# electrum/presto

Measured on AMD Instinct MI355X. Metric: rows/s through operator pipeline, TPC-H Q1+Q6 SF100, 1/2/4/8 GPUs vs CPU ref, higher is better.
Workload: dtype f64

## Files before the change

### presto_amd/csrc/op_fused.cpp

```cpp
#include <algorithm>
#include <cstring>
#include <sstream>

#include "op_fused.hpp"

namespace pa {
namespace fused_op {

FusedAggregationOperator::FusedAggregationOperator(const pa_fused_aggregation_desc* d)
    : FusedAggregationOperator(make_spec(d), d->aggregation.stream ? d->aggregation.stream : d->filter_project.stream)
{
}

FusedAggregationOperator::FusedAggregationOperator(Spec spec, void* stream) : spec_(std::move(spec)), stream_(stream)
{
    require_device();
    nullable_seen_.assign(spec_.n_in, false);
    out_partial_ = spec_.step == PA_STEP_PARTIAL;
    {
        std::ostringstream f;
        for (int c = 0; c < spec_.n_in; c++) f << spec_.in_types[c] << ',' << spec_.in_params[c] << ';';
        f << '|' << (spec_.has_filter ? spec_.filter.fingerprint() : std::string("-")) << '|';
        for (const auto& p : spec_.proj) f << p.fingerprint() << '#';
        f << '|';
        for (int g : spec_.group_proj) f << g << ',';
        f << '|' << spec_.hash_channel << '|' << spec_.step << '|';
        for (const auto& a : spec_.aggs) f << a.fn << ',' << a.input_channel << ',' << a.mask_channel << ',' << a.input_type << ';';
        if (spec_.join) {
            f << "|join:" << spec_.join->key_proj << ':';
            for (int32_t t : spec_.join->build_types) f << t << ',';
            f << ':';
            for (int j : spec_.join->brow_group_proj) f << j << ',';
        }
        f << "|lds_pipe:" << lds_pipe_level();
        plan_fingerprint_ = f.str();
    }
    grouped_ = !spec_.group_proj.empty();
    mode_ = grouped_ ? (spec_.expected_groups > (1 << 20) ? V_GT : V_LDS) : V_GLOBAL;
    if (spec_.any_ranked() && grouped_) mode_ = V_GT;
    cus_ = device_cu_count();
    ctl_ = static_cast<int32_t*>(ctl_buf_.ensure(64));
    PA_HIP(hipMemsetAsync(ctl_, 0, 64, stream_.get()));
    h_ctl_ = static_cast<int32_t*>(h_ctl_buf_.ensure(256));
    memset(h_ctl_, 0, 256);
}

FusedAggregationOperator::~FusedAggregationOperator()
{
    (void)hipStreamSynchronize(stream_.get());
    if (lds_.merge_stream) pool_stream_release(lds_.merge_stream);
    release_everything();
    for (hipEvent_t e : release_events_) (void)hipEventDestroy(e);
    for (int b = 0; b < 2; b++) {
        if (arena_[b].table_event) (void)hipEventDestroy(arena_[b].table_event);
        if (arena_[b].vtable_event) (void)hipEventDestroy(arena_[b].vtable_event);
        if (lds_.ev_main[b]) (void)hipEventDestroy(lds_.ev_main[b]);
        if (lds_.ev_merge[b]) (void)hipEventDestroy(lds_.ev_merge[b]);
    }
    for (RangeTable& t : range_table_) {
        if (t.event) (void)hipEventDestroy(t.event);
    }
}

bool FusedAggregationOperator::set_output_topn(int64_t n, const int32_t* channels, const int32_t* orders, int32_t count)
{
    if (n <= 0 || count <= 0 || !grouped_ || out_partial_ || spec_.step == PA_STEP_PARTIAL) return false;
    topn_hint_.n = n;
    topn_hint_.channels.assign(channels, channels + count);
    topn_hint_.orders.assign(orders, orders + count);
    return true;
}

bool FusedAggregationOperator::retry_parked()
{
    if (!parked_) return true;
    if (!pool_has_room(parked_need_)) return false;
    parked_ = false;
    pa_page page = parked_page_;
    page.columns = parked_cols_.data();
    take_page(&page);
    return !parked_;
}

void FusedAggregationOperator::take_page(const pa_page* page)
{
    const uint64_t launched = timer.begun();
    try {
        if (next_) {
            next_->add_input(page);
            return;
        }
        cur_rel_set_ = (page->flags & PA_PAGE_RETAINED) != 0 && page->release != nullptr;
        cur_rel_ = Release{page->release, page->release_ctx};
        if (gather_small_page(page)) return;
        flush_pending();
        if (next_) {
            cur_rel_set_ = false;
            next_->add_input(page);
            return;
        }
        process_page(page, page_stays(page) && page->mem == PA_MEM_DEVICE);
        if (cur_rel_set_) {
            std::vector<Release> rel{cur_rel_};
            cur_rel_set_ = false;
            release_checkpoint(std::move(rel), true);
        }
    }
    catch (const PoolExhausted& e) {
        if (!page_stays(page) || timer.begun() != launched || is_combiner_) throw;
        parked_page_ = *page;
        if (!cur_rel_set_) parked_page_.flags &= ~PA_PAGE_RETAINED;
        cur_rel_set_ = false;
        parked_cols_.assign(page->columns, page->columns + page->channel_count);
        parked_need_ = e.bytes;
        parked_ = true;
    }
}

void FusedAggregationOperator::add_input(const pa_page* page)
{
    PA_REQUIRE(!finishing_, PA_ERR_ILLEGAL_STATE, "Operator is already finishing");
    PA_REQUIRE(page != nullptr, PA_ERR_INVALID_ARGUMENT, "page is null");
    PA_REQUIRE(page->channel_count == spec_.n_in, PA_ERR_INVALID_ARGUMENT, "page channel count does not match the operator's input types");
    poll_releases();
    if (page->position_count == 0) {
        if ((page->flags & PA_PAGE_RETAINED) != 0 && page->release) page->release(page->release_ctx);
        return;
    }
    PA_REQUIRE(!parked_, PA_ERR_ILLEGAL_STATE, "Operator has unfinished work");
    take_page(page);
}

void FusedAggregationOperator::process_page(const pa_page* page, bool retained)
{
    if (next_) {
        next_->process_page(page, retained);
        return;
    }
    retained_ = retained;
    try {
        add_page(page);
    }
    catch (const LayoutChange&) {
        start_next_generation();
        next_->process_page(page, retained);
    }
    retained_ = false;
}

void FusedAggregationOperator::start_next_generation()
{
    PA_REQUIRE(!is_combiner_ && generation_ <= spec_.n_in, PA_ERR_DEVICE, "internal: state layout changed more often than channels exist");
    confirm_all();
    next_ = std::make_unique<FusedAggregationOperator>(spec_, stream_.get());
    next_->nullable_seen_ = nullable_seen_;
    next_->generation_ = generation_ + 1;
}

void FusedAggregationOperator::finish()
{
    if (finishing_) return;
    PA_REQUIRE(retry_parked(), PA_ERR_INSUFFICIENT_RESOURCES, "finish while a page is still waiting for HBM: the pool's budget does not cover the aggregation");
    flush_pending();
    finishing_ = true;
    poll_releases();
}

bool FusedAggregationOperator::get_output(pa_page* out)
{
    poll_releases();
    if (!finishing_ || output_done_) return false;
    output_done_ = true;
    confirm_all();
    if (next_) return combine_generations(out);
    build_output();
    if (grouped_ && out_rows_ > 0) decode_interned_keys();
    if (!grouped_ || out_rows_ > 0) {
        publish_output(out_cols_, out_rows_, spec_.output_mem, stream_.get(), out, out_storage_);
        poll_releases();
        return true;
    }
    poll_releases();
    return false;
}

bool FusedAggregationOperator::emit_states(pa_page* out)
{
    flush_pending();
    confirm_all();
    out_partial_ = true;
    spec_.output_mem = PA_MEM_DEVICE;
    build_output();
    if (grouped_ && out_rows_ > 0) decode_interned_keys();
    if (grouped_ && out_rows_ == 0) return false;
    publish_output(out_cols_, out_rows_, PA_MEM_DEVICE, stream_.get(), out, out_storage_);
    return true;
}

bool FusedAggregationOperator::combine_generations(pa_page* out)
{
    Spec cs = combiner_spec();
    combiner_ = std::make_unique<FusedAggregationOperator>(std::move(cs), stream_.get());
    combiner_->out_partial_ = spec_.step == PA_STEP_PARTIAL;
    combiner_->nullable_seen_.assign(combiner_->spec_.n_in, true);
    combiner_->is_combiner_ = true;
    for (FusedAggregationOperator* g = this; g != nullptr; g = g->next_.get()) {
        pa_page states{};
        if (g->emit_states(&states)) combiner_->add_input(&states);
    }
    combiner_->finish();
    return combiner_->get_output(out);
}

Spec FusedAggregationOperator::combiner_spec() const
{
    Spec c;
    c.step = PA_STEP_FINAL;
    c.output_mem = spec_.output_mem;
    c.expected_groups = spec_.expected_groups;
    auto add_channel = [&](int32_t type, int32_t param) {
        c.in_types.push_back(type);
        c.in_params.push_back(param);
        OwnedExpr e;
        pa_expr_node node{};
        node.kind = PA_EXPR_INPUT_REF;
        node.type = type;
        node.channel = c.n_in;
        e.nodes.push_back(node);
        e.strings.emplace_back();
        e.root = 0;
        c.proj.push_back(std::move(e));
        return c.n_in++;
    };
    for (size_t gi = 0; gi < spec_.group_proj.size(); gi++) {
        const OwnedExpr& pe = spec_.proj[spec_.group_proj[gi]];
        int ch = pe.is_input_ref() ? pe.node(pe.root).channel : -1;
        if (ch >= spec_.n_in) ch = -1;
        const bool interned = ch >= 0 && spec_.interned[ch];
        c.group_proj.push_back(add_channel(interned ? (int32_t)PA_VARCHAR : pe.root_type(), ch >= 0 ? spec_.in_params[ch] : 0));
    }
    c.hash_channel = spec_.hash_channel >= 0 && !spec_.group_proj.empty() ? add_channel(PA_BIGINT, 0) : -1;
    for (const pa_aggregate& ag : spec_.aggs) {
        pa_aggregate f = ag;
        f.mask_channel = -1;
        f.input_channel = add_channel(PA_BIGINT, 0);
        if (ag.fn != PA_AGG_COUNT && ag.fn != PA_AGG_COUNT_STAR) {
            const int value_proj = spec_.step == PA_STEP_FINAL ? ag.input_channel + 1 : ag.input_channel;
            int32_t t = spec_.proj[value_proj].root_type();
            if (ag.fn == PA_AGG_AVG || (ag.fn == PA_AGG_SUM && t == PA_DOUBLE)) t = PA_DOUBLE;
// ... 180 lines not shown
```

### presto_amd/csrc/op_fused.hpp

```cpp
#pragma once

#include <atomic>
#include <deque>
#include <map>
#include <memory>
#include <mutex>
#include <string>
#include <vector>

#include "exchange_kernels.hpp"
#include "fused_plan.hpp"
#include "intern_kernels.hpp"
#include "jit.hpp"
#include "join_source.hpp"
#include "operator.hpp"
#include "scan_kernels.hpp"
#include "static_kernels.hpp"

namespace pa {

using namespace fused;

namespace fused_op {

// ... 29 lines not shown
        if (!retry_parked()) return true;
        if (next_) return next_->is_blocked();
        poll_inflight();
        return lds_.inflight.size() >= kMaxInflight;
    }
    void add_input(const pa_page* page) override;
    void finish() override;
    bool is_finished() override { return finishing_ && output_done_; }
    bool get_output(pa_page* out) override;
    bool set_output_topn(int64_t n, const int32_t* channels, const int32_t* orders, int32_t count) override;
    int64_t memory_bytes() override
    {
        return (int64_t)(stager_.bytes() + slab_.capacity() + gt_.tag.capacity() + gt_.keys.capacity() + gt_.words.capacity() + state_.capacity());
    }
    int64_t group_bytes();
    const Spec& spec() const { return spec_; }
    void* stream_handle() { return stream_.get(); }

private:
    struct TopNHint {
        int64_t n = 0;
        std::vector<int32_t> channels, orders;
    };
    struct Release {
        void (*fn)(void*) = nullptr;
        void* ctx = nullptr;
    };
    struct ReleaseBatch {
        hipEvent_t event = nullptr;
        uint64_t seq = 0;
        std::vector<Release> rel;
    };
    struct Compiled {
        KernelInfo info;
        JitKernel kernel, tail_kernel;
        DevBuf kinds;
        mutable std::atomic<int> lds_verdict{0};
        mutable std::atomic<int> staged_verdict{0};
    };
    struct RowList {
        const int32_t* rows;
        int64_t count;
        int64_t first_row;
        int64_t chunk_rows;
    };
    struct Inflight {
        int b = 0;
        DevPage dp;
        bool vec = false;
        int64_t offset = 0;
        std::string sig;
        std::vector<ChannelLayout> layout;
        uint64_t seq = 0;
    };
    struct Run {
        int64_t rows = 0;
        bool flat = true;
        std::vector<pa_column> cols;
    };
    struct RangeTable {
        PinnedBuf host;
        DevBuf dev;
        hipEvent_t event = nullptr;
        bool used = false;
    };
    struct Arena {
        int64_t rows = 0;
        std::vector<bool> nullable;
        std::vector<DevBuf> values, nulls, offsets;
        std::vector<int64_t> bytes;
        std::vector<CopySeg> segs;
        std::vector<Release> rel;
        PinnedBuf h_table;
        DevBuf d_table;
        hipEvent_t table_event = nullptr;
        bool table_used = false;
        bool dev_var = false, var_fresh = true;
        int cursor_half = 0;
        DevBuf cursors;
        std::vector<VarSeg> vsegs;
        PinnedBuf h_vtable;
        DevBuf d_vtable;
        hipEvent_t vtable_event = nullptr;
        bool vtable_used = false;
    };
    struct RankedChannel {
        std::vector<std::string> strings;
        std::vector<uint32_t> order;
        DevBuf ranks, image;
    };

    bool lookup_source_ready() const { return !spec_.join || spec_.join->ls->built.load(); }
    static bool page_stays(const pa_page* page) { return (page->flags & (PA_PAGE_STABLE | PA_PAGE_RETAINED)) != 0; }
    bool retry_parked();
    void take_page(const pa_page* page);
    void process_page(const pa_page* page, bool retained);
    void start_next_generation();
    bool emit_states(pa_page* out);
    bool combine_generations(pa_page* out);
    Spec combiner_spec() const;
    static void raise_if(int32_t code);

    Release take_cur_release()
    {
        cur_rel_set_ = false;
        return cur_rel_;
// ... 33 lines not shown
    static std::mutex& shared_mutex();
    static std::map<std::string, std::shared_ptr<const Compiled>>& shared_cache();
    const Compiled& kernel_for(const std::string& sig, const std::vector<ChannelLayout>& layout, int variant);
    void adopt_layout(const Compiled& c);
    static constexpr int64_t kStagedMinRows = (int64_t)1 << 22;
    static constexpr double kStagedGain = 0.85;
    static int staged_mode();
    const Compiled* staged_kernel(const std::string& sig, const std::vector<ChannelLayout>& layout, int64_t rows);
    static double staged_bytes(const std::vector<int>& w, const std::vector<double>& alive);
    void staged_decide(const Compiled& ck, const uint64_t* slab, int grid, int64_t vec_rows, hipStream_t s);
    bool run_page(const Compiled& ck, const DevPage& dp, bool vec, const RowList* list = nullptr, int64_t start_row = 0);
    void fill_join_args(FusedArgs& a) const;
    void advance_columns(FusedArgs& a, const DevPage& dp, int64_t offset) const;
    bool run_page_build_rows(const Compiled& ck, const DevPage& dp, FusedArgs a, int64_t start_row);
    bool launch_global(const Compiled& ck, const DevPage& dp, FusedArgs& a, int64_t offset, int64_t total, int64_t range_entries);
    bool launch_lds(const Compiled& ck, const DevPage& dp, FusedArgs& a, bool vec, int64_t offset, int64_t total, int64_t range_entries);
    bool launch_table(const Compiled& ck, const DevPage& dp, FusedArgs& a, const RowList* list, int64_t offset, int64_t total);
    int grid_for(const KernelInfo& ki, int64_t work, const RowList* list) const;
    uint32_t replicas_for(const KernelInfo& ki, int grid, const RowList* list) const;
    FusedArgs replay_args(const FusedArgs& a, uint32_t spilled, int cur, uint64_t flush_room);
    static constexpr size_t kMaxInflight = 2;
    int32_t* h_ctl_lds(int b) const { return h_ctl_ + 16 + 8 * b; }
    void poll_inflight();
    void confirm_all();
    void confirm_all_but_last();
    bool confirm_oldest(bool redo = true);

    static constexpr int64_t kProbeRows = (int64_t)1 << 18;
    static constexpr uint32_t kLdshReplicas = 4;
    static uint32_t desired_replicas(uint64_t g);
    void ensure_table(uint64_t min_groups, uint32_t reps = 0);
    static uint64_t estimate_groups(uint64_t d, uint64_t n);
    void drop_table();
    void read_group_counts(hipStream_t s);
    void drain_merges();
    bool partitioned_wanted(const std::string& sig, const std::vector<ChannelLayout>& layout, int* partitions);
    void run_page_partitioned(const std::string& sig, const std::vector<ChannelLayout>& layout, const DevPage& dp, bool vec, int partitions,
                              int64_t start_row);
    const uint64_t* table_tags() const
    {
        return build_rows_table_ && brow_occ_word_ >= 0 ? gt_.words.as<uint64_t>() + (size_t)brow_occ_word_ * gt_.cap : gt_.tag.as<uint64_t>();
    }
    const uint64_t* table_words() const { return gt_.words.as<uint64_t>(); }
    GtStrides table_strides() const { return GtStrides{1u, gt_.cap, 1u, 0u, build_rows_table_ && brow_occ_word_ >= 0 ? brow_occ_empty_ : 0ULL}; }

    void intern_keys(DevPage& dp, hipStream_t s);
    void intern_dictionary_key(const pa_page* page, int c, DevPage& dp, hipStream_t s);
    void decode_interned_keys();
    int interned_channel(int gi) const;
    void rank_values(DevPage& dp, hipStream_t s);
    void rerank_words(int c, const uint32_t* ranks, hipStream_t s);
    int ranked_channel(int proj) const;

    void build_output();
    bool emit_on_device(const KernelInfo& ki, int64_t groups, bool keys_from_build_columns = false);


    Spec spec_;
    Stream stream_;
    std::string plan_fingerprint_;
    bool grouped_ = false, finishing_ = false, output_done_ = false;
    int cus_ = 256;
    int mode_ = V_GLOBAL;
    DevBuf ctl_buf_;
    PinnedBuf h_ctl_buf_;
    int32_t* ctl_ = nullptr;
    int32_t* h_ctl_ = nullptr;

    TopNHint topn_hint_;
    bool out_partial_ = false;
    std::vector<bool> nullable_seen_;
    int generation_ = 0;
    bool is_combiner_ = false;
    std::unique_ptr<FusedAggregationOperator> next_;
    std::unique_ptr<FusedAggregationOperator> combiner_;
    bool parked_ = false;
    pa_page parked_page_{};
    std::vector<pa_column> parked_cols_;
    size_t parked_need_ = 0;

    PageStager stager_;
    PinnedPageCopy pinned_copy_;
    std::vector<int64_t> var_bytes_hint_;
    Release cur_rel_;
    bool cur_rel_set_ = false;
    std::vector<Release> run_rel_, ranges_rel_, carry_rel_;
    std::deque<ReleaseBatch> release_batches_;
    std::vector<hipEvent_t> release_events_;
    Run run_;
    std::shared_ptr<std::vector<DevPage>> ranges_;
    int64_t range_rows_ = 0;
    RangeTable range_table_[3];
    int range_table_next_ = 0;
    Arena arena_[2];
    int arena_cur_ = 0;

    std::map<std::string, std::shared_ptr<const Compiled>> compiled_;
    bool layout_fixed_ = false;
    int nw_ = 0, w_ = 0;
    std::string layout_id_;
    const int32_t* kinds_dev_ = nullptr;
    const KernelInfo* last_info_ = nullptr;
    bool staged_refused_ = false;
    bool join_checked_ = false;
    const std::string* cur_sig_ = nullptr;
    const std::vector<ChannelLayout>* cur_layout_ = nullptr;
    bool retained_ = false;
    int64_t resume_from_ = -1;

    DevBuf slab_, state_;

    struct LdsTier {
        DevBuf slab[2], entry_slot[2];
        hipStream_t merge_stream = nullptr;
        hipEvent_t ev_main[2] = {nullptr, nullptr}, ev_merge[2] = {nullptr, nullptr};
        bool merge_pending[2] = {false, false};
        int page = 0;
        bool probed = false;
        const Compiled* compiled = nullptr;
        std::deque<Inflight> inflight;
        uint64_t launch_seq = 0;
    } lds_;

    struct HbmTable {
        DevBuf tag, keys, words, rep_count, spill[2];
        PinnedBuf h_rep;
        uint32_t cap = 0, rep = 1;
        uint64_t groups_upper = 0, groups_sum = 0;
        uint64_t probed_groups = 0;
        bool probed = false;
    } gt_;
    bool build_rows_table_ = false;
    const Compiled* brow_keys_ = nullptr;
    int brow_occ_word_ = -1;
    uint64_t brow_occ_empty_ = 0;

    struct Partitioned {
        int parts = 0, lc = 0;
        bool want = false;
        bool fresh = false;
        uint64_t fell = 0;
        DevBuf tag, keys, words, count, part_first;
        DevBuf part_ids, part_pos, part_counts, part_temp;
        std::vector<DevBuf> reorder_bufs;
        int list_grid_hint = 0;
    } ldsp_;

    std::vector<std::unique_ptr<StringInterner>> interners_;
    PageStager dict_stager_;
    std::vector<DevBuf> dict_key_bufs_;
    std::vector<std::unique_ptr<RankedChannel>> ranked_;

    PinnedBuf h_table_, h_parts_;
    DevBuf dense_keys_, dense_words_, null_flags_;
    std::vector<OutColumn> out_cols_;
    std::vector<pa_column> out_storage_;
    int32_t out_rows_ = 0;
    static constexpr int64_t kHostDecodeGroups = 4096;
    static constexpr uint32_t kHostDecodeIds = 4096;
    std::vector<std::vector<std::string>> host_dict_;
};

}
}
```

### presto_amd/csrc/op_fused_launch.cpp

```cpp
#include <algorithm>
#include <cmath>
#include <cstring>

#include "op_fused.hpp"

namespace pa {
namespace fused_op {

void FusedAggregationOperator::add_page(const pa_page* page)
{
    HostTraceScope trace("  fused.add_page");
    hipStream_t s = stream_.get();
    std::vector<int> dict_keys;
    std::vector<bool> needed = spec_.used_channel;
    for (int c = 0; c < spec_.n_in; c++) {
        if (!spec_.interned[c]) continue;
        const pa_column& col = page->columns[c];
        const bool encoded = (col.encoding == PA_DICTIONARY && col.ids != nullptr) || col.encoding == PA_RLE;
        if (!encoded || col.dictionary == nullptr || col.dictionary->encoding != PA_VARWIDTH) continue;
        const int64_t dn = col.encoding == PA_RLE ? 1 : col.dictionary_size;
        if (dn <= 0 || dn > page->position_count) continue;
        needed[c] = false;
        dict_keys.push_back(c);
    }
// ... 212 lines not shown
    return true;
}

bool FusedAggregationOperator::launch_lds(const Compiled& ck, const DevPage& dp, FusedArgs& a, bool vec, int64_t offset, int64_t total,
                                          int64_t range_entries)
{
    hipStream_t s = stream_.get();
    const KernelInfo& ki = ck.info;
    const int64_t lds_head = dp.ranges ? total : vec ? (total & ~(int64_t)255) : 0;
    while (offset < total) {
        int64_t n = total - offset;
        bool use_tail = false;
        if (offset < lds_head) {
            n = lds_head - offset;
            if (!lds_.probed && ck.lds_verdict.load(std::memory_order_relaxed) == 1) lds_.probed = true;
            lds_.compiled = &ck;
            if (!lds_.probed && n > ((int64_t)1 << 22) && !dp.ranges) n = (int64_t)1 << 20;
        }
        else use_tail = true;
        advance_columns(a, dp, offset);
        a.n = n;
        int64_t work = use_tail ? n : (n + 3) / 4;
        if (dp.ranges) work = range_entries * ki.block;
        const int per_cu = std::max(1, std::min(16, (int)(160 * 1024 / ((size_t)ki.nw * ki.c * 64 * 8 + 512))));
        const int grid = std::max((int)std::min<int64_t>((work + 63) / 64, (int64_t)cus_ * per_cu), 1);
        const int b = lds_.page & 1;
        if (!lds_.merge_stream) {
            lds_.merge_stream = pool_stream_acquire();
            for (int i = 0; i < 2; i++) {
                PA_HIP(hipEventCreateWithFlags(&lds_.ev_main[i], hipEventDisableTiming));
                PA_HIP(hipEventCreateWithFlags(&lds_.ev_merge[i], hipEventDisableTiming));
            }
        }
        while (lds_.inflight.size() >= kMaxInflight) confirm_oldest();
        if (mode_ != V_LDS) {
            resume_from_ = offset;
            return false;
        }
        if (lds_.merge_pending[b]) PA_HIP(hipStreamWaitEvent(s, lds_.ev_merge[b], 0));
        a.slab = static_cast<uint64_t*>(lds_.slab[b].ensure((size_t)grid * ki.c * (1 + ki.w + ki.nw) * 8));
        a.overflow_rows = reinterpret_cast<uint64_t*>(ctl_ + 2 + 2 * b);
        ensure_table(gt_.groups_upper + 2 * (uint64_t)grid * ki.c);
        a.gt_tag = gt_.tag.as<uint64_t>();
        a.gt_keys = gt_.keys.as<uint64_t>();
        a.gt_words = gt_.words.as<uint64_t>();
        a.gt_mask = gt_.cap ? gt_.cap - 1 : 0;
        a.gt_max_fill = (int32_t)(gt_.cap - gt_.cap / 4);
        a.gt_rep_count = gt_.rep_count.as<int32_t>();
        void* params[] = {&a};
        if (!use_tail) timer.set_name(ck.kernel.name);
        timer.begin(s);
        PA_HIP(hipModuleLaunchKernel(use_tail ? ck.tail_kernel.fn : ck.kernel.fn, grid, 1, 1, ki.block, 1, 1, 0, s, params, nullptr));
        timer.end(s, !use_tail);
        PA_HIP(hipMemcpyAsync(h_ctl_lds(b), ctl_, 32, hipMemcpyDeviceToHost, s));
        PA_HIP(hipEventRecord(lds_.ev_main[b], s));
        PA_HIP(hipStreamWaitEvent(lds_.merge_stream, lds_.ev_main[b], 0));
        launch_merge_lds_slab(a.slab, grid, ki.c, ki.w, ki.nw, ck.kinds.as<int32_t>(), a.gt_tag, a.gt_keys, a.gt_words, a.gt_mask,
                              a.gt_max_fill, a.gt_count, ctl_, a.overflow_rows,
                              static_cast<int32_t*>(lds_.entry_slot[b].ensure((size_t)grid * ki.c * 4)), lds_.merge_stream);
        PA_HIP(hipEventRecord(lds_.ev_merge[b], lds_.merge_stream));
        lds_.merge_pending[b] = true;
        lds_.page++;
        Inflight f;
        f.b = b;
        f.dp = dp;
        f.dp.n = (int32_t)(offset + n);
        f.vec = vec;
        f.offset = offset;
        f.sig = *cur_sig_;
        f.layout = *cur_layout_;
        f.seq = ++lds_.launch_seq;
        lds_.inflight.push_back(std::move(f));
        if (!lds_.probed) {
            confirm_all_but_last();
            if (!confirm_oldest(false)) {
                resume_from_ = offset;
                return false;
            }
        }
        else if (!retained_) confirm_all();
        else poll_inflight();
        if (mode_ != V_LDS) {
            resume_from_ = offset + n;
            return false;
        }
        offset += n;
        if (resume_from_ >= 0) return false;
    }
    return true;
}

int FusedAggregationOperator::grid_for(const KernelInfo& ki, int64_t work, const RowList* list) const
{
    int grid;
    if (ki.variant == V_LDSP) {
        grid = ldsp_.parts;
    }
    else if (ki.variant == V_LDSH) {
        grid = (int)std::min<int64_t>((work + ki.block - 1) / ki.block, (int64_t)cus_ * (ki.block == 1024 ? 1 : 2));
        if (list && ldsp_.list_grid_hint > grid) grid = (int)std::min<int64_t>((work + ki.block - 1) / ki.block, (int64_t)ldsp_.list_grid_hint);
    }
    else {
        grid = (int)std::min<int64_t>((work + 255) / 256, (int64_t)cus_ * 8);
    }
    return std::max(grid, 1);
}

uint32_t FusedAggregationOperator::replicas_for(const KernelInfo& ki, int grid, const RowList* list) const
{
    if (ki.variant == V_LDSP) return gt_.rep;
    uint32_t want = desired_replicas(gt_.probed ? gt_.groups_upper : std::max<uint64_t>(gt_.groups_upper, (uint64_t)std::max(spec_.expected_groups, 1)));
    if (ki.variant == V_LDSH) want = std::min<uint32_t>(want, kLdshReplicas);
    uint32_t reps = (want >= 2 * gt_.rep || want * 4 <= gt_.rep) ? want : gt_.rep;
    reps = std::min<uint32_t>(reps, next_pow2((uint64_t)grid));
    if (ki.variant == V_LDSH && !gt_.probed && !list && gt_.groups_upper == 0) reps = 1;
    return reps;
}

FusedArgs FusedAggregationOperator::replay_args(const FusedArgs& a, uint32_t spilled, int cur, uint64_t flush_room)
{
    FusedArgs r = a;
    r.n = 0;
    if (r.list_blocked == 2) r.list_blocked = 1;
    r.row_list = gt_.spill[cur].as<int32_t>();
// ... 72 lines not shown
            raise_if(h_ctl_[0]);
            const bool first_probe = !gt_.probed;
            gt_.probed = true;
            const uint32_t spilled = (uint32_t)h_ctl_[6];
            if (ki.variant == V_LDSP) {
                uint64_t fell;
                memcpy(&fell, h_ctl_ + 2, 8);
                if (fell != 0) PA_HIP(hipMemsetAsync(ctl_ + 2, 0, 8, s));
                ldsp_.fell += fell;
            }
            if (ki.variant == V_LDSH) {
                uint64_t fell;
                memcpy(&fell, h_ctl_ + 2, 8);
                if (fell != 0) PA_HIP(hipMemsetAsync(ctl_ + 2, 0, 8, s));
                if (fell > (uint64_t)n / 4) mode_ = V_GT;
                if (lone_probe && first_probe && estimate_groups(gt_.groups_sum, (uint64_t)n) > (uint64_t)ki.lc / 2) mode_ = V_GT;
            }
            if (spilled == 0) {
                if (ki.variant == V_LDSH && mode_ == V_GT && !list && offset + n < total) resume_from_ = offset + n;
                if (ki.variant == V_GT && first_probe && !list && offset + n < total && mode_ == V_GT) {
                    int p = 0;
                    if (partitioned_wanted(*cur_sig_, *cur_layout_, &p)) resume_from_ = offset + n;
                }
                if (lone_probe && resume_from_ >= 0 && mode_ == V_GT && !getenv("PRESTO_AMD_KEEP_PROBE")) {
                    int p = 0;
                    gt_.probed_groups = std::max(gt_.probed_groups, estimate_groups(gt_.groups_sum, (uint64_t)n));
                    if (partitioned_wanted(*cur_sig_, *cur_layout_, &p) && ldsp_.want) {
                        drop_table();
                        resume_from_ = offset;
                    }
                }
                break;
            }
            PA_HIP(hipMemsetAsync(ctl_ + 6, 0, 4, s));
            ensure_table(std::max<uint64_t>((uint64_t)gt_.cap / 2 + 1, gt_.groups_upper + spilled) + flush_room);
            FusedArgs r = replay_args(a, spilled, cur, flush_room);
            void* rparams[] = {&r};
            const Compiled& rk = ki.variant == V_LDSP ? kernel_for(*cur_sig_, *cur_layout_, V_GT) : ck;
            int rgrid = (int)std::max<int64_t>(1, std::min<int64_t>(((int64_t)spilled + rk.info.block - 1) / rk.info.block, (int64_t)grid));
            timer.begin(s);
            PA_HIP(hipModuleLaunchKernel(rk.kernel.fn, rgrid, 1, 1, rk.info.block, 1, 1, 0, s, rparams, nullptr));
            timer.end(s);
            cur ^= 1;
        }
        offset += n;
        if (resume_from_ >= 0) return false;
    }
    return true;
}


void FusedAggregationOperator::poll_inflight()
{
    while (!lds_.inflight.empty() && hipEventQuery(lds_.ev_main[lds_.inflight.front().b]) == hipSuccess) confirm_oldest();
    (void)hipGetLastError();
}

void FusedAggregationOperator::confirm_all()
{
    while (!lds_.inflight.empty()) confirm_oldest();
}

void FusedAggregationOperator::confirm_all_but_last()
{
    while (lds_.inflight.size() > 1) confirm_oldest();
}

bool FusedAggregationOperator::confirm_oldest(bool redo)
{
    Inflight f = std::move(lds_.inflight.front());
    lds_.inflight.pop_front();
    PA_HIP(hipEventSynchronize(lds_.ev_main[f.b]));
    const int32_t* hc = h_ctl_lds(f.b);
    uint64_t overflow;
    memcpy(&overflow, hc + 2 + 2 * f.b, 8);
    raise_if(hc[0]);
    if (overflow == 0) {
        gt_.groups_upper = std::max<uint64_t>(gt_.groups_upper, (uint64_t)hc[1]);
        lds_.probed = true;
        if (lds_.compiled) lds_.compiled->lds_verdict.store(1, std::memory_order_relaxed);
        return true;
    }
    if (lds_.compiled) lds_.compiled->lds_verdict.store(2, std::memory_order_relaxed);
    hipStream_t s = stream_.get();
    drain_merges();
    PA_HIP(hipMemsetAsync(ctl_ + 2 + 2 * f.b, 0, 8, s));
    if (mode_ == V_LDS) mode_ = V_LDSH;
    if (!redo) return false;
    const int64_t saved = resume_from_;
    const bool saved_retained = retained_;
    retained_ = false;
    run_tiers(f.sig, f.layout, f.dp, f.vec, f.offset);
    retained_ = saved_retained;
    resume_from_ = saved;
    return false;
}

}
}
```

### presto_amd/csrc/op_fused_output.cpp

```cpp
#include <algorithm>
#include <cstring>

#include "decimal_host.hpp"
#include "host_hash.hpp"
#include "op_fused.hpp"
#include "topn_kernels.hpp"

namespace pa {
namespace fused_op {

bool FusedAggregationOperator::emit_on_device(const KernelInfo& ki, int64_t groups, bool keys_from_build_columns)
{
    constexpr int64_t kMinGroups = 4096;
    const int nkeys = (int)spec_.group_proj.size();
    const bool has_hash = nkeys > 0 && spec_.hash_channel >= 0;
    const bool partial = out_partial_;
    if (groups < kMinGroups || groups > INT32_MAX) return false;
    if (spec_.any_ranked()) return false;
    for (int gi = 0; gi < nkeys; gi++) {
        if (ki.keys[gi].type == PA_VARCHAR || ki.keys[gi].type == PA_DECIMAL) return false;
    }
    for (size_t k = 0; k < spec_.aggs.size(); k++) {
        if (ki.agg_limbs[k] > 0) return false;
        const int value_proj = spec_.step == PA_STEP_FINAL ? spec_.aggs[k].input_channel + 1 : spec_.aggs[k].input_channel;
// ... 89 lines not shown
    for (int c = 0; c < n; c++) {
        OutColumn& oc = out_cols_[c];
        oc.type = a.col[c].type;
        a.col[c].values = oc.values.ensure((size_t)groups * a.col[c].width);
        a.col[c].nulls = nullable[c] ? static_cast<uint8_t*>(oc.nulls.ensure((size_t)groups)) : nullptr;
    }
    a.tag = table_tags();
    a.keys = gt_.keys.as<uint64_t>();
    a.words = table_words();
    a.st = table_strides();
    a.cap = gt_.cap;
    a.W = std::max(w_, 1);
    a.NW = nw_;
    a.ncols = n;
    a.counter = reinterpret_cast<uint32_t*>(ctl_ + 7);
    a.null_flags = static_cast<uint32_t*>(null_flags_.ensure(GT_EMIT_MAX_COLS * 4));
    DevBuf topn_keys;
    bool bounded = false;
    if (topn_hint_.n > 0 && !partial && groups >= (int64_t)1 << 16 && groups >= 64 * topn_hint_.n) {
        const int c0 = topn_hint_.channels[0];
        const int64_t cap = (int64_t)gt_.cap;
        constexpr int64_t kSample = (int64_t)1 << 14;
        const double j = (double)topn_hint_.n * (double)kSample / (double)cap;
        const int64_t rank = (int64_t)std::ceil(j + 8.0 + 4.0 * std::sqrt(j));
        if (c0 >= 0 && c0 < n && a.col[c0].kind != GT_EMIT_HASH && cap >= 4 * kSample && rank <= kSample / 8) {
            uint64_t* keys = static_cast<uint64_t*>(topn_keys.ensure((size_t)kSample * 8 + 64));
            uint64_t* bound = keys + kSample;
            launch_gt_emit_keys_strided(a, c0, topn_hint_.orders[0], cap / kSample, kSample, keys, s);
            launch_topn_sample_bound(PA_TOPN_KEYS, keys, nullptr, nullptr, kSample, 1, kSample, rank, nullptr, bound, s);
            a.filter_bound = bound;
            a.filter_col = c0;
            a.filter_order = topn_hint_.orders[0];
            bounded = true;
        }
    }
    uint32_t flags[GT_EMIT_MAX_COLS];
    for (;;) {
        PA_HIP(hipMemsetAsync(ctl_ + 7, 0, 4, s));
        PA_HIP(hipMemsetAsync(a.null_flags, 0, GT_EMIT_MAX_COLS * 4, s));
        launch_gt_emit(a, s);
        PA_HIP(hipMemcpyAsync(h_ctl_, ctl_, 32, hipMemcpyDeviceToHost, s));
        read_back(flags, a.null_flags, sizeof(flags), s);
        if (!bounded || (int64_t)(uint32_t)h_ctl_[7] >= topn_hint_.n) break;
        bounded = false;
        a.filter_bound = nullptr;
    }
    if (keys_from_build_columns || bounded) groups = (int64_t)(uint32_t)h_ctl_[7];
    PA_REQUIRE((int64_t)(uint32_t)h_ctl_[7] == groups, PA_ERR_DEVICE, "group table and group count disagree");
    for (int c = 0; c < n; c++) out_cols_[c].has_nulls = flags[c] != 0;
    out_rows_ = (int32_t)groups;
    return true;
}

void FusedAggregationOperator::build_output()
{
    HostTraceScope trace("  fused.build_output");
    hipStream_t s = stream_.get();
    drain_merges();
    if (compiled_.empty()) {
        std::vector<ChannelLayout> layout(spec_.n_in);
        for (int c = 0; c < spec_.n_in; c++) layout[c].type = spec_.in_types[c];
        auto c = std::make_shared<Compiled>();
        c->info = generate(spec_, layout, grouped_ ? V_GT : V_GLOBAL);
        nw_ = c->info.nw;
        w_ = c->info.w;
        compiled_["-"] = std::move(c);
    }
    const KernelInfo& ki = compiled_.begin()->second->info;

    const bool sub_tables = grouped_ && ldsp_.parts > 0;
    const int32_t* per_part = nullptr;
    if (sub_tables) {
        per_part = static_cast<const int32_t*>(h_parts_.ensure((size_t)ldsp_.parts * 4));
        PA_HIP(hipMemcpyAsync(h_parts_.ptr(), ldsp_.count.ptr(), (size_t)ldsp_.parts * 4, hipMemcpyDeviceToHost, s));
        read_group_counts(s);
    }
    else {
        PA_HIP(hipMemcpyAsync(h_ctl_, ctl_, 32, hipMemcpyDeviceToHost, s));
        PA_HIP(hipStreamSynchronize(s));
    }
    raise_if(h_ctl_[0]);
    if (sub_tables) {
        uint64_t total = 0;
        for (int p = 0; p < ldsp_.parts; p++) total += (uint64_t)per_part[p];
        const uint32_t sub_cap = (uint32_t)ldsp_.parts * (uint32_t)ldsp_.lc;
        if (gt_.groups_sum == 0) {
            gt_.tag = std::move(ldsp_.tag);
            gt_.keys = std::move(ldsp_.keys);
            gt_.words = std::move(ldsp_.words);
            gt_.cap = sub_cap;
            gt_.rep = 1;
            h_ctl_[1] = (int32_t)total;
            PA_HIP(hipMemcpyAsync(ctl_ + 1, h_ctl_ + 1, 4, hipMemcpyHostToDevice, s));
            gt_.groups_upper = gt_.groups_sum = total;
        }
        else {
            ensure_table(gt_.groups_sum + total + 1024, 1);
            launch_gt_fold(ldsp_.tag.as<uint64_t>(), ldsp_.keys.as<uint64_t>(), ldsp_.words.as<uint64_t>(), sub_cap, 1, std::max(w_, 1), nw_, kinds_dev_,
                           gt_.tag.as<uint64_t>(), gt_.keys.as<uint64_t>(), gt_.words.as<uint64_t>(), gt_.cap - 1, 1, ctl_ + 1, gt_.rep_count.as<int32_t>(), ctl_, s);
            PA_HIP(hipMemcpyAsync(h_ctl_, ctl_, 32, hipMemcpyDeviceToHost, s));
            PA_HIP(hipStreamSynchronize(s));
            raise_if(h_ctl_[0]);
            ldsp_.tag.release();
            ldsp_.keys.release();
            ldsp_.words.release();
        }
        ldsp_.parts = 0;
    }
    std::vector<uint64_t> keys, words;
    int64_t groups = 0;
    if (!grouped_) {
        groups = 1;
        words.assign(nw_, 0);
        if (state_.ptr()) PA_HIP(hipMemcpy(words.data(), state_.ptr(), (size_t)nw_ * 8, hipMemcpyDeviceToHost));
    }
    else if (gt_.cap > 0) {
        if (gt_.rep > 1) {
            read_group_counts(s);
            ensure_table(gt_.groups_sum, 1);
            PA_HIP(hipMemcpyAsync(h_ctl_, ctl_, 32, hipMemcpyDeviceToHost, s));
            PA_HIP(hipStreamSynchronize(s));
            raise_if(h_ctl_[0]);
        }
        if (build_rows_table_ && (int64_t)gt_.cap >= (1 << 14) && emit_on_device(ki, (int64_t)gt_.cap, true)) return;
        if (build_rows_table_) {
            FusedArgs a;
            memset(&a, 0, sizeof a);
            fill_join_args(a);
            a.err = ctl_;
            a.gt_count = ctl_ + 1;
            PA_HIP(hipMemsetAsync(ctl_ + 1, 0, 4, s));
            a.gt_tag = gt_.tag.as<uint64_t>();
            a.gt_keys = gt_.keys.as<uint64_t>();
            a.gt_words = gt_.words.as<uint64_t>();
            a.gt_mask = gt_.cap - 1;
            void* params[] = {&a};
            const int grid = (int)std::max<int64_t>(1, std::min<int64_t>(((int64_t)gt_.cap + 255) / 256, (int64_t)cus_ * 8));
            PA_HIP(hipModuleLaunchKernel(brow_keys_->tail_kernel.fn, grid, 1, 1, 256, 1, 1, 0, s, params, nullptr));
            PA_HIP(hipMemcpyAsync(h_ctl_, ctl_, 32, hipMemcpyDeviceToHost, s));
            PA_HIP(hipStreamSynchronize(s));
            raise_if(h_ctl_[0]);
        }
        groups = h_ctl_[1];
        if (emit_on_device(ki, groups)) return;
        if (groups > 0) {
            const int kw = std::max(w_, 1);
            dense_keys_.ensure((size_t)groups * kw * 8);
            dense_words_.ensure((size_t)groups * nw_ * 8);
            PA_HIP(hipMemsetAsync(ctl_ + 7, 0, 4, s));
            const GtStrides st = table_strides();
            launch_gt_compact(table_tags(), gt_.keys.as<uint64_t>(), table_words(), gt_.cap, kw, nw_, dense_keys_.as<uint64_t>(),
                              dense_words_.as<uint64_t>(), reinterpret_cast<uint32_t*>(ctl_ + 7), s, &st);
            uint8_t* land = static_cast<uint8_t*>(h_table_.ensure((size_t)groups * (kw + nw_) * 8));
            PA_HIP(hipMemcpyAsync(land, dense_keys_.ptr(), (size_t)groups * kw * 8, hipMemcpyDeviceToHost, s));
            PA_HIP(hipMemcpyAsync(land + (size_t)groups * kw * 8, dense_words_.ptr(), (size_t)groups * nw_ * 8, hipMemcpyDeviceToHost, s));
            PA_HIP(hipStreamSynchronize(s));
            const uint64_t* hk = reinterpret_cast<const uint64_t*>(land);
            const uint64_t* hw = hk + (size_t)groups * kw;
            keys.resize((size_t)groups * w_);
            for (int64_t g = 0; g < groups; g++) {
                for (int w = 0; w < w_; w++) keys[(size_t)g * w_ + w] = hk[(size_t)g * kw + w];
            }
            words.assign(hw, hw + (size_t)groups * nw_);
        }
    }
    PA_REQUIRE(groups <= INT32_MAX, PA_ERR_INSUFFICIENT_RESOURCES, "too many groups for one output page");
    out_rows_ = (int32_t)groups;

    const int nkeys = (int)spec_.group_proj.size();
    const bool has_hash = nkeys > 0 && spec_.hash_channel >= 0;
    const bool partial = out_partial_;
    int agg_cols = 0;
    for (const auto& ag : spec_.aggs) agg_cols += (partial && ag.fn != PA_AGG_COUNT && ag.fn != PA_AGG_COUNT_STAR) ? 2 : 1;
    const int ncols = nkeys + (has_hash ? 1 : 0) + agg_cols;
    out_cols_.clear();
    out_cols_.resize(ncols);
    std::vector<std::vector<uint8_t>> host_cols(ncols), host_nulls(ncols);
    std::vector<std::vector<int32_t>> host_offsets(ncols);
    std::vector<int64_t> row_hash(groups, 0);
    int col = 0;
    for (int gi = 0; gi < nkeys; gi++, col++) {
        const KeyPart& kp = ki.keys[gi];
        OutColumn& oc = out_cols_[col];
        std::vector<uint64_t> dict_hash;
        const int ic = interned_channel(gi);
        if (ic >= 0 && has_hash && groups > 0 && !interners_.empty() && interners_[ic] && interners_[ic]->size()) {
            dict_hash.resize(interners_[ic]->size());
            PA_HIP(hipMemcpyAsync(dict_hash.data(), interners_[ic]->hashes(), dict_hash.size() * 8, hipMemcpyDeviceToHost, s));
            PA_HIP(hipStreamSynchronize(s));
        }
        const std::vector<std::string>* host_dict = nullptr;
        if (ic >= 0 && spec_.output_mem != PA_MEM_DEVICE && groups > 0 && groups <= kHostDecodeGroups && !interners_.empty() && interners_[ic] &&
            interners_[ic]->size() <= kHostDecodeIds) {
            if (host_dict_.empty()) host_dict_.resize(spec_.n_in);
            interners_[ic]->fetch_strings((uint32_t)host_dict_[ic].size(), &host_dict_[ic], s);
            host_dict = &host_dict_[ic];
        }
        oc.type = host_dict ? PA_VARCHAR : kp.type;
        oc.varwidth = oc.type == PA_VARCHAR;
        auto& data = host_cols[col];
        auto& nulls = host_nulls[col];
        auto& offs = host_offsets[col];
        nulls.assign(groups ? groups : 1, 0);
        bool any_null = false;
        if (oc.varwidth) offs.push_back(0);
        const uint64_t mask = kp.bits >= 64 ? ~0ULL : ((1ULL << kp.bits) - 1ULL);
        for (int64_t g = 0; g < groups; g++) {
            const uint64_t* kw = &keys[(size_t)g * w_];
            bool is_null = kp.null_word >= 0 && ((kw[kp.null_word] >> kp.null_shift) & 1ULL);
            int64_t h = 0;
            if (is_null) {
                nulls[g] = 1;
                any_null = true;
            }
            uint64_t w0 = (kw[kp.word] >> kp.shift) & mask;
            switch (kp.type) {
                case PA_BIGINT:
                case PA_DECIMAL: {
// ... 253 lines not shown
                        double avg = sum / (double)count;
                        memcpy(&bits, &avg, 8);
                    }
                    break;
                default:
                    break;
            }
            if (width == 8) memcpy(&data[(size_t)g * 8], &bits, 8);
            else if (real_out) {
                double d;
                memcpy(&d, &bits, 8);
                const float f = (float)d;
                memcpy(&data[(size_t)g * 4], &f, 4);
            }
            else {
                int32_t v = (int32_t)(int64_t)bits;
                memcpy(&data[(size_t)g * 4], &v, 4);
            }
        }
        oc.has_nulls = any_null;
        col++;
    }
    const bool to_device = spec_.output_mem == PA_MEM_DEVICE;
    for (int c = 0; c < ncols; c++) {
        OutColumn& oc = out_cols_[c];
        size_t bytes = host_cols[c].size();
        void* hv = oc.h_values.ensure(bytes ? bytes : 1);
        if (bytes) memcpy(hv, host_cols[c].data(), bytes);
        if (oc.varwidth) {
            void* ho = oc.h_offsets.ensure(host_offsets[c].size() * 4);
            memcpy(ho, host_offsets[c].data(), host_offsets[c].size() * 4);
        }
        if (oc.has_nulls) {
            void* hn = oc.h_nulls.ensure(host_nulls[c].size());
            memcpy(hn, host_nulls[c].data(), host_nulls[c].size());
        }
        oc.host_ready = true;
        if (to_device) {
            oc.values.ensure(bytes ? bytes : 1);
            if (bytes) PA_HIP(hipMemcpyAsync(oc.values.ptr(), hv, bytes, hipMemcpyHostToDevice, s));
            if (oc.varwidth) {
                oc.offsets.ensure(host_offsets[c].size() * 4);
                PA_HIP(hipMemcpyAsync(oc.offsets.ptr(), oc.h_offsets.ptr(), host_offsets[c].size() * 4, hipMemcpyHostToDevice, s));
            }
            if (oc.has_nulls) {
                oc.nulls.ensure(host_nulls[c].size());
                PA_HIP(hipMemcpyAsync(oc.nulls.ptr(), oc.h_nulls.ptr(), host_nulls[c].size(), hipMemcpyHostToDevice, s));
            }
        }
    }
    if (to_device) PA_HIP(hipStreamSynchronize(s));
}

}
}
```

Baseline: 207.1 billion.

## Enqueue eager aggregation result readback at finish and defer LDS control copy

At finish, small aggregations (ungrouped or few groups) now queue the table compaction and the device-to-host copy of the results right away. get_output can then use the pinned landing buffer instead of draining merges and doing synchronous readbacks. The LDS control-word copy is moved onto the merge stream for retained pages once the kernel has been probed, and the destructor waits on a recorded event rather than the whole stream. The goal is to cut sync round-trips at output time, at the cost of extra validation logic and possibly wasted compaction when the eager result does not hold.

```diff
diff --git a/presto_amd/csrc/op_fused.cpp b/presto_amd/csrc/op_fused.cpp
--- a/presto_amd/csrc/op_fused.cpp
+++ b/presto_amd/csrc/op_fused.cpp
@@ -43,13 +43,17 @@
     PA_HIP(hipMemsetAsync(ctl_, 0, 64, stream_.get()));
     h_ctl_ = static_cast<int32_t*>(h_ctl_buf_.ensure(256));
     memset(h_ctl_, 0, 256);
+    if (const char* e = getenv("PRESTO_AMD_EAGER_OUTPUT")) eager_.on = atoi(e) != 0;
 }
 
 FusedAggregationOperator::~FusedAggregationOperator()
 {
-    (void)hipStreamSynchronize(stream_.get());
+    if (!stream_.owned() && last_event_ && last_valid_) (void)hipEventSynchronize(last_event_);
+    else (void)hipStreamSynchronize(stream_.get());
     if (lds_.merge_stream) pool_stream_release(lds_.merge_stream);
     release_everything();
+    if (last_event_) (void)hipEventDestroy(last_event_);
+    if (eager_.event) (void)hipEventDestroy(eager_.event);
     for (hipEvent_t e : release_events_) (void)hipEventDestroy(e);
     for (int b = 0; b < 2; b++) {
         if (arena_[b].table_event) (void)hipEventDestroy(arena_[b].table_event);
@@ -85,6 +89,7 @@
 void FusedAggregationOperator::take_page(const pa_page* page)
 {
     const uint64_t launched = timer.begun();
+    last_valid_ = false;
     try {
         if (next_) {
             next_->add_input(page);
@@ -161,9 +166,19 @@
 {
     if (finishing_) return;
     PA_REQUIRE(retry_parked(), PA_ERR_INSUFFICIENT_RESOURCES, "finish while a page is still waiting for HBM: the pool's budget does not cover the aggregation");
+    last_valid_ = false;
     flush_pending();
     finishing_ = true;
     poll_releases();
+    mark_last_event();
+    if (eager_possible()) enqueue_eager_result();
+}
+
+void FusedAggregationOperator::mark_last_event()
+{
+    if (!last_event_) PA_HIP(hipEventCreateWithFlags(&last_event_, hipEventDisableTiming));
+    PA_HIP(hipEventRecord(last_event_, stream_.get()));
+    last_valid_ = true;
 }
 
 bool FusedAggregationOperator::get_output(pa_page* out)
@@ -171,30 +186,34 @@
     poll_releases();
     if (!finishing_ || output_done_) return false;
     output_done_ = true;
-    confirm_all();
-    if (next_) return combine_generations(out);
-    build_output();
+    const bool eager = eager_result_holds();
+    if (!eager) {
+        last_valid_ = false;
+        confirm_all();
+        if (next_) return combine_generations(out);
+    }
+    build_output(eager);
     if (grouped_ && out_rows_ > 0) decode_interned_keys();
-    if (!grouped_ || out_rows_ > 0) {
-        publish_output(out_cols_, out_rows_, spec_.output_mem, stream_.get(), out, out_storage_);
-        poll_releases();
-        return true;
-    }
+    const bool any = !grouped_ || out_rows_ > 0;
+    if (any) publish_output(out_cols_, out_rows_, spec_.output_mem, stream_.get(), out, out_storage_);
+    if (!eager) mark_last_event();
     poll_releases();
-    return false;
+    return any;
 }
 
 bool FusedAggregationOperator::emit_states(pa_page* out)
 {
+    last_valid_ = false;
     flush_pending();
     confirm_all();
     out_partial_ = true;
     spec_.output_mem = PA_MEM_DEVICE;
     build_output();
     if (grouped_ && out_rows_ > 0) decode_interned_keys();
-    if (grouped_ && out_rows_ == 0) return false;
-    publish_output(out_cols_, out_rows_, PA_MEM_DEVICE, stream_.get(), out, out_storage_);
-    return true;
+    const bool any = !grouped_ || out_rows_ > 0;
+    if (any) publish_output(out_cols_, out_rows_, PA_MEM_DEVICE, stream_.get(), out, out_storage_);
+    mark_last_event();
+    return any;
 }
 
 bool FusedAggregationOperator::combine_generations(pa_page* out)
diff --git a/presto_amd/csrc/op_fused.hpp b/presto_amd/csrc/op_fused.hpp
--- a/presto_amd/csrc/op_fused.hpp
+++ b/presto_amd/csrc/op_fused.hpp
@@ -105,6 +105,7 @@
         std::string sig;
         std::vector<ChannelLayout> layout;
         uint64_t seq = 0;
+        bool late_ctl = false;
     };
     struct Run {
         int64_t rows = 0;
@@ -244,8 +245,17 @@
     void rerank_words(int c, const uint32_t* ranks, hipStream_t s);
     int ranked_channel(int proj) const;
 
-    void build_output();
+    void build_output(bool eager = false);
+    bool fetch_result(const KernelInfo& ki, std::vector<uint64_t>& keys, std::vector<uint64_t>& words, int64_t& groups);
+    void assemble_output(const KernelInfo& ki, const std::vector<uint64_t>& keys, const std::vector<uint64_t>& words, int64_t groups);
     bool emit_on_device(const KernelInfo& ki, int64_t groups, bool keys_from_build_columns = false);
+    static constexpr int64_t kEagerGroups = 1024;
+    static constexpr uint32_t kEagerTableSlots = 1u << 20;
+    bool eager_possible() const;
+    void enqueue_eager_result();
+    bool eager_result_holds();
+    void take_eager_result(std::vector<uint64_t>& keys, std::vector<uint64_t>& words, int64_t& groups) const;
+    void mark_last_event();
 
 
     Spec spec_;
@@ -343,6 +353,18 @@
     std::vector<DevBuf> dict_key_bufs_;
     std::vector<std::unique_ptr<RankedChannel>> ranked_;
 
+    struct Eager {
+        bool on = true;
+        bool queued = false;
+        hipEvent_t event = nullptr;
+        bool with_state = false;
+        size_t rows = 0;
+        uint64_t begun = 0;
+        PinnedBuf land;
+    } eager_;
+    hipEvent_t last_event_ = nullptr;
+    bool last_valid_ = false;
+
     PinnedBuf h_table_, h_parts_;
     DevBuf dense_keys_, dense_words_, null_flags_;
     std::vector<OutColumn> out_cols_;
diff --git a/presto_amd/csrc/op_fused_launch.cpp b/presto_amd/csrc/op_fused_launch.cpp
--- a/presto_amd/csrc/op_fused_launch.cpp
+++ b/presto_amd/csrc/op_fused_launch.cpp
@@ -288,12 +288,14 @@
         timer.begin(s);
         PA_HIP(hipModuleLaunchKernel(use_tail ? ck.tail_kernel.fn : ck.kernel.fn, grid, 1, 1, ki.block, 1, 1, 0, s, params, nullptr));
         timer.end(s, !use_tail);
-        PA_HIP(hipMemcpyAsync(h_ctl_lds(b), ctl_, 32, hipMemcpyDeviceToHost, s));
+        const bool late_ctl = lds_.probed && retained_;
+        if (!late_ctl) PA_HIP(hipMemcpyAsync(h_ctl_lds(b), ctl_, 32, hipMemcpyDeviceToHost, s));
         PA_HIP(hipEventRecord(lds_.ev_main[b], s));
         PA_HIP(hipStreamWaitEvent(lds_.merge_stream, lds_.ev_main[b], 0));
         launch_merge_lds_slab(a.slab, grid, ki.c, ki.w, ki.nw, ck.kinds.as<int32_t>(), a.gt_tag, a.gt_keys, a.gt_words, a.gt_mask,
                               a.gt_max_fill, a.gt_count, ctl_, a.overflow_rows,
                               static_cast<int32_t*>(lds_.entry_slot[b].ensure((size_t)grid * ki.c * 4)), lds_.merge_stream);
+        if (late_ctl) PA_HIP(hipMemcpyAsync(h_ctl_lds(b), ctl_, 32, hipMemcpyDeviceToHost, lds_.merge_stream));
         PA_HIP(hipEventRecord(lds_.ev_merge[b], lds_.merge_stream));
         lds_.merge_pending[b] = true;
         lds_.page++;
@@ -306,6 +308,7 @@
         f.sig = *cur_sig_;
         f.layout = *cur_layout_;
         f.seq = ++lds_.launch_seq;
+        f.late_ctl = late_ctl;
         lds_.inflight.push_back(std::move(f));
         if (!lds_.probed) {
             confirm_all_but_last();
@@ -484,7 +487,11 @@
 
 void FusedAggregationOperator::poll_inflight()
 {
-    while (!lds_.inflight.empty() && hipEventQuery(lds_.ev_main[lds_.inflight.front().b]) == hipSuccess) confirm_oldest();
+    while (!lds_.inflight.empty()) {
+        const Inflight& f = lds_.inflight.front();
+        if (hipEventQuery(f.late_ctl ? lds_.ev_merge[f.b] : lds_.ev_main[f.b]) != hipSuccess) break;
+        confirm_oldest();
+    }
     (void)hipGetLastError();
 }
 
@@ -502,7 +509,7 @@
 {
     Inflight f = std::move(lds_.inflight.front());
     lds_.inflight.pop_front();
-    PA_HIP(hipEventSynchronize(lds_.ev_main[f.b]));
+    PA_HIP(hipEventSynchronize(f.late_ctl ? lds_.ev_merge[f.b] : lds_.ev_main[f.b]));
     const int32_t* hc = h_ctl_lds(f.b);
     uint64_t overflow;
     memcpy(&overflow, hc + 2 + 2 * f.b, 8);
@@ -515,6 +522,7 @@
     }
     if (lds_.compiled) lds_.compiled->lds_verdict.store(2, std::memory_order_relaxed);
     hipStream_t s = stream_.get();
+    last_valid_ = false;
     drain_merges();
     PA_HIP(hipMemsetAsync(ctl_ + 2 + 2 * f.b, 0, 8, s));
     if (mode_ == V_LDS) mode_ = V_LDSH;
diff --git a/presto_amd/csrc/op_fused_output.cpp b/presto_amd/csrc/op_fused_output.cpp
--- a/presto_amd/csrc/op_fused_output.cpp
+++ b/presto_amd/csrc/op_fused_output.cpp
@@ -165,11 +165,10 @@
     return true;
 }
 
-void FusedAggregationOperator::build_output()
+void FusedAggregationOperator::build_output(bool eager)
 {
     HostTraceScope trace("  fused.build_output");
-    hipStream_t s = stream_.get();
-    drain_merges();
+    if (!eager) drain_merges();
     if (compiled_.empty()) {
         std::vector<ChannelLayout> layout(spec_.n_in);
         for (int c = 0; c < spec_.n_in; c++) layout[c].type = spec_.in_types[c];
@@ -180,7 +179,16 @@
         compiled_["-"] = std::move(c);
     }
     const KernelInfo& ki = compiled_.begin()->second->info;
-
+    std::vector<uint64_t> keys, words;
+    int64_t groups = 0;
+    if (eager) take_eager_result(keys, words, groups);
+    else if (!fetch_result(ki, keys, words, groups)) return;
+    assemble_output(ki, keys, words, groups);
+}
+
+bool FusedAggregationOperator::fetch_result(const KernelInfo& ki, std::vector<uint64_t>& keys, std::vector<uint64_t>& words, int64_t& groups)
+{
+    hipStream_t s = stream_.get();
     const bool sub_tables = grouped_ && ldsp_.parts > 0;
     const int32_t* per_part = nullptr;
     if (sub_tables) {
@@ -220,8 +228,6 @@
         }
         ldsp_.parts = 0;
     }
-    std::vector<uint64_t> keys, words;
-    int64_t groups = 0;
     if (!grouped_) {
         groups = 1;
         words.assign(nw_, 0);
@@ -235,7 +241,7 @@
             PA_HIP(hipStreamSynchronize(s));
             raise_if(h_ctl_[0]);
         }
-        if (build_rows_table_ && (int64_t)gt_.cap >= (1 << 14) && emit_on_device(ki, (int64_t)gt_.cap, true)) return;
+        if (build_rows_table_ && (int64_t)gt_.cap >= (1 << 14) && emit_on_device(ki, (int64_t)gt_.cap, true)) return false;
         if (build_rows_table_) {
             FusedArgs a;
             memset(&a, 0, sizeof a);
@@ -255,7 +261,7 @@
             raise_if(h_ctl_[0]);
         }
         groups = h_ctl_[1];
-        if (emit_on_device(ki, groups)) return;
+        if (emit_on_device(ki, groups)) return false;
         if (groups > 0) {
             const int kw = std::max(w_, 1);
             dense_keys_.ensure((size_t)groups * kw * 8);
@@ -277,6 +283,12 @@
             words.assign(hw, hw + (size_t)groups * nw_);
         }
     }
+    return true;
+}
+
+void FusedAggregationOperator::assemble_output(const KernelInfo& ki, const std::vector<uint64_t>& keys, const std::vector<uint64_t>& words, int64_t groups)
+{
+    hipStream_t s = stream_.get();
     PA_REQUIRE(groups <= INT32_MAX, PA_ERR_INSUFFICIENT_RESOURCES, "too many groups for one output page");
     out_rows_ = (int32_t)groups;
 
@@ -636,5 +648,85 @@
     if (to_device) PA_HIP(hipStreamSynchronize(s));
 }
 
-}
-}
+
+bool FusedAggregationOperator::eager_possible() const
+{
+    if (!eager_.on || next_ || is_combiner_ || parked_) return false;
+    if (ldsp_.parts > 0 || gt_.rep > 1 || build_rows_table_ || topn_hint_.n > 0) return false;
+    if (spec_.output_mem == PA_MEM_DEVICE || spec_.any_ranked()) return false;
+    for (int c = 0; c < spec_.n_in; c++) {
+        if (spec_.interned[c]) return false;
+    }
+    return !grouped_ || (gt_.cap <= kEagerTableSlots && gt_.groups_upper <= (uint64_t)kEagerGroups);
+}
+
+void FusedAggregationOperator::enqueue_eager_result()
+{
+    hipStream_t s = stream_.get();
+    if (lds_.merge_stream) {
+        s = lds_.merge_stream;
+        PA_HIP(hipStreamWaitEvent(s, last_event_, 0));
+    }
+    if (!eager_.event) PA_HIP(hipEventCreateWithFlags(&eager_.event, hipEventDisableTiming));
+    const size_t kw = (size_t)std::max(w_, 1), nw = (size_t)nw_;
+    eager_.with_state = !grouped_ && state_.ptr() != nullptr;
+    eager_.rows = grouped_ && gt_.cap > 0 ? (size_t)std::min<int64_t>(kEagerGroups, (int64_t)gt_.cap) : 0;
+    uint8_t* land = static_cast<uint8_t*>(eager_.land.ensure(32 + (grouped_ ? eager_.rows * (kw + nw) : nw) * 8));
+    if (eager_.rows > 0) {
+        dense_keys_.ensure((size_t)gt_.cap * kw * 8);
+        dense_words_.ensure(std::max<size_t>((size_t)gt_.cap * nw * 8, 8));
+        PA_HIP(hipMemsetAsync(ctl_ + 7, 0, 4, s));
+        const GtStrides st = table_strides();
+        launch_gt_compact(table_tags(), gt_.keys.as<uint64_t>(), table_words(), gt_.cap, (int)kw, nw_, dense_keys_.as<uint64_t>(),
+                          dense_words_.as<uint64_t>(), reinterpret_cast<uint32_t*>(ctl_ + 7), s, &st);
+    }
+    PA_HIP(hipMemcpyAsync(land, ctl_, 32, hipMemcpyDeviceToHost, s));
+    if (eager_.with_state && nw > 0) PA_HIP(hipMemcpyAsync(land + 32, state_.ptr(), nw * 8, hipMemcpyDeviceToHost, s));
+    if (eager_.rows > 0) {
+        PA_HIP(hipMemcpyAsync(land + 32, dense_keys_.ptr(), eager_.rows * kw * 8, hipMemcpyDeviceToHost, s));
+        if (nw > 0) PA_HIP(hipMemcpyAsync(land + 32 + eager_.rows * kw * 8, dense_words_.ptr(), eager_.rows * nw * 8, hipMemcpyDeviceToHost, s));
+    }
+    PA_HIP(hipEventRecord(eager_.event, s));
+    if (s == stream_.get()) mark_last_event();
+    eager_.begun = timer.begun();
+    eager_.queued = true;
+}
+
+bool FusedAggregationOperator::eager_result_holds()
+{
+    if (!eager_.queued) return false;
+    eager_.queued = false;
+    PA_HIP(hipEventSynchronize(eager_.event));
+    confirm_all();
+    if (timer.begun() != eager_.begun || next_) return false;
+    const int32_t* ctl = eager_.land.as<int32_t>();
+    raise_if(ctl[0]);
+    if (!grouped_) return true;
+    const int64_t groups = ctl[1];
+    if (groups == 0) return true;
+    return groups <= (int64_t)eager_.rows && (int64_t)(uint32_t)ctl[7] == groups;
+}
+
+void FusedAggregationOperator::take_eager_result(std::vector<uint64_t>& keys, std::vector<uint64_t>& words, int64_t& groups) const
+{
+    const uint8_t* land = eager_.land.as<uint8_t>();
+    if (!grouped_) {
+        groups = 1;
+        words.assign(nw_, 0);
+        if (eager_.with_state && nw_ > 0) memcpy(words.data(), land + 32, (size_t)nw_ * 8);
+        return;
+    }
+    groups = reinterpret_cast<const int32_t*>(land)[1];
+    if (groups == 0) return;
+    const int kw = std::max(w_, 1);
+    const uint64_t* hk = reinterpret_cast<const uint64_t*>(land + 32);
+    const uint64_t* hw = hk + eager_.rows * (size_t)kw;
+    keys.resize((size_t)groups * w_);
+    for (int64_t g = 0; g < groups; g++) {
+        for (int w = 0; w < w_; w++) keys[(size_t)g * w_ + w] = hk[(size_t)g * kw + w];
+    }
+    words.assign(hw, hw + (size_t)groups * nw_);
+}
+
+}
+}
```

Result: faster. 215.7 billion (median of 6 runs) (+4.2%).
